# Luh1124/face-vae

Hardware: AMD Instinct MI355X
Metric: training images/sec (256x256 face-VAE step) (higher is better)
Workload: dtype bf16; 1 GPU; FaceVAE step 256x256 (AFE trunk + reparam + Generator trunk, MSE+KL, Adam); global_batch=32, per_gpu_batch=32, resolution=256, parallelism=dp1

## Files before the change

### face-vae_amd/_lib.py

```python
from __future__ import annotations

import ctypes
import os
from ctypes import POINTER, c_float, c_int, c_long, c_size_t, c_void_p

import torch

_HERE = os.path.dirname(os.path.realpath(__file__))
LIB_PATH = os.environ.get("FV_LIB_PATH") or os.path.join(_HERE, "libfacevae.so")

FV_F32, FV_BF16, FV_F64 = 0, 1, 2
FV_E_BADARG, FV_E_UNSUPPORTED, FV_E_COMM = 1001, 1002, 1003
ADAM_CHUNK = 4096
ABI_VERSION = 2


class ConvDesc(ctypes.Structure):
    _fields_ = [
        ("dtype", c_int), ("n", c_int), ("h", c_int), ("w", c_int),
        ("cin", c_int), ("cin_valid", c_int), ("cout", c_int), ("ldy", c_int),
        ("ksize", c_int), ("upsample", c_int), ("pro_act", c_int), ("pro_slope", c_float),
        ("epi_sigmoid", c_int), ("out_nchw_f32", c_int),
    ]

# ... 40 lines not shown
    "fv_conv_wt_elems": (c_size_t, [D]),
    "fv_conv2d_stats_blocks": (c_int, [D]),
    "fv_conv2d_stats_block_pixels": (c_int, [D]),
    "fv_conv_weight_prep": (c_int, [D, P, P, P, P, P]),
    "fv_conv2d_fwd": (c_int, [D, P, P, P, P, P, P, P, P, P]),
    "fv_conv2d_bwd_data": (c_int, [D, P, c_int, P, P, P]),
    "fv_conv2d_dgrad_lowres": (c_int, [D]),
    "fv_conv2d_wgrad_nsplit": (c_int, [D]),
    "fv_conv2d_wgrad_slab_elems": (c_size_t, [D]),
    "fv_conv2d_wgrad_bias_slab_elems": (c_size_t, [D]),
    "fv_conv2d_bwd_weight": (c_int, [D, P, P, P, P, c_int, P, P, P]),
    "fv_conv2d_wgrad_reduce": (c_int, [D, P, P, P, P, P]),
    "fv_conv2d_sr_records": (c_int, [D, c_int, POINTER(c_int)]),
    "fv_conv2d_fwd_sr": (c_int, [D, P, P, P, P, P, P, P]),
    "fv_conv2d_bwd_data_sr": (c_int, [D, P, c_int, P, P, P, P]),
    "fv_bn_bwd_from_records": (c_int, [P, c_int, c_int, c_long, c_int, c_long, P, P, P, P, P, P]),
    "fv_convt_supported": (c_int, [D]),
    "fv_convt_weight_prep": (c_int, [D, P, c_int, c_float, P, P, P, P]),
    "fv_convt_wgrad_reduce": (c_int, [D, P, P, P, c_int, c_float, P, P, P, P]),
    "fv_convt_eff_weight": (c_int, [P, c_int, c_int, c_int, c_int, c_float, P, P, P]),
    "fv_convt_weight_grad": (c_int, [P, c_int, c_int, c_int, c_int, c_float, P, P, P]),
    "fv_convt_direct_fwd": (c_int, [c_int, P, c_int, c_int, c_int, c_int, c_int, P, P, c_int, c_int, c_int, c_int,
                                    c_int, P, P]),
    "fv_convt_direct_dgrad": (c_int, [c_int, P, c_int, c_int, c_int, c_int, c_int, P, c_int, c_int, c_int, c_int,
                                      c_int, P, P]),
    "fv_convt_direct_wgrad": (c_int, [c_int, P, P, c_int, c_int, c_int, c_int, c_int, c_int, c_int, c_int, c_int,
                                      c_int, P, P, P]),
    "fv_chan_scale_fwd": (c_int, [c_int, P, c_int, c_long, c_int, c_int, P, P, P, P]),
    "fv_chan_scale_bwd": (c_int, [c_int, P, P, c_int, c_long, c_int, c_int, P, P, P, P, P]),
    "fv_fp8_ws_bytes": (c_size_t, []),
# ... 315 lines not shown
```

### face-vae_amd/csrc/conv.hip

```cpp
#include "conv_plan.h"

namespace {

__global__ void weight_prep_c7n_kernel(const float* __restrict__ wp, const float* sigma, bf16* wn, int cout) {
  const float inv = sigma ? 1.f / sigma[0] : 1.f;
  for (int e = blockIdx.x * blockDim.x + threadIdx.x; e < 32 * 448; e += gridDim.x * blockDim.x) {
    const int nn = e / 448, k = e - nn * 448;
    const int co = nn / 7, s = nn - co * 7, r = k >> 6, ci = k & 63;
    const float v = co < cout ? wp[((co * 64 + ci) * 7 + r) * 7 + s] * inv : 0.f;
    wn[e] = (bf16)v;
  }
}

template <typename T>
__device__ __forceinline__ void weight_prep_body(const float* __restrict__ wp, const float* sigma, T* wk, int rows,
                                                 int Kpad, int cout, int cin_valid, int lgCin, int KS, int K,
                                                 int transposed, int bid, int nblk, int smaj = 0) {
  const int total = rows * Kpad;
  const float inv = sigma ? 1.f / sigma[0] : 1.f;
  for (int e = bid * (int)blockDim.x + threadIdx.x; e < total; e += nblk * (int)blockDim.x) {
    int row, k;
    bool kin;
    int tap, c;
    if (smaj == 2) {
// ... 843 lines not shown
  }
  const bool c64 = use_c64(d);
  if (c64 && !res && !a.spm) {
    if ((st = wext(d->cout, kpad_of(3, 64), "c64"))) return st;
    const int nb = c64_bands(d);
    const int nblk = d->n * (d->w / 64) * (d->cout / 64) * nb;
    const unsigned xb = (unsigned)((long)d->n * d->h * d->w * 64 * 2);
    launch_c64(a, nblk, xb, nb, s);
    return fv_check_launch("conv2d_fwd_c64");
  }
  if (use_c74(d)) {
    FV_REQUIRE(!res, "packed 7x7 conv: no residual");
    const int ntiles = d->n * (d->h / C74_TR) * (d->w / 64);
    const unsigned xb = (unsigned)((long)d->n * d->h * d->w * d->cin * 2);
    FV_REQUIRE(!a.stats || a.nrec == c74_grid(d), "packed 7x7 conv: %d BN records for %d blocks", a.nrec, c74_grid(d));
    launch_c74(a, c74_grid(d), xb, ntiles, s);
    return fv_check_launch("conv2d_fwd_c74");
  }
  if (const int tr = halo_tr(d)) {
    if ((st = wext(plan_tile(d).bn, kpad_of(7, d->cin), "halo7"))) return st;
    a.lgtw = 6;
    const int nblk = d->n * (d->h / tr) * (d->w / 64);
    const unsigned xb = (unsigned)((long)d->n * d->h * d->w * d->cin * 2);
    if (launch_halo7(a, d->cin, nblk, xb, s)) {
      fv_set_error("7x7 halo conv variant unsupported (cin=%d)", d->cin);
      return FV_E_BADARG;
    }
    return fv_check_launch("conv2d_fwd_halo");
  }
  if (use_upband(d)) {
    FV_REQUIRE(!res && !a.spm, "sub-pixel band conv: no residual / store-pass records");
// ... 124 lines not shown
  return conv_run(d, x, wk, bias, pro_scale, pro_shift, res, y, stats, (hipStream_t)stream);
}

static fv_conv_desc dgrad_desc(const fv_conv_desc* d) {
  fv_conv_desc t{};
  t.dtype = d->dtype;
  t.n = d->n; t.h = d->h; t.w = d->w;
  t.cin = pad_pow2_8(d->cout);
  t.cin_valid = d->cout;
  t.cout = d->cin;
  t.ldy = d->cin;
  t.ksize = d->ksize;
  return t;
}

int fv_conv2d_sr_records(const fv_conv_desc* d, int dgrad, int* record_pixels) {
  if (check_desc(d) != FV_OK) return 0;
  if (dgrad) {
    if (d->upsample) return 0;
    const fv_conv_desc t = dgrad_desc(d);
    return sr_geometry(&t, record_pixels);
  }
  return sr_geometry(d, record_pixels);
}

int fv_conv2d_fwd_sr(const fv_conv_desc* d, const void* x, const void* wk, const float* bias, const void* res, void* y,
                     const fv_store_reduce* sr, void* stream) {
  int st = check_desc(d);
  if (st) return st;
  FV_REQUIRE(x && wk && y && sr && sr->mode == 1, "fwd_sr: null pointer or mode != 1");
  FV_REQUIRE(!d->pro_act && !d->out_nchw_f32 && d->ldy == d->cout, "fwd_sr: plain NHWC output only");
  return conv_run(d, x, wk, bias, nullptr, nullptr, res, y, nullptr, (hipStream_t)stream, sr);
}

int fv_conv2d_bwd_data_sr(const fv_conv_desc* d, const void* dy, int ldy_dy, const void* wt, void* dx,
                          const fv_store_reduce* sr, void* stream) {
  int st = check_desc(d);
  if (st) return st;
  FV_REQUIRE(dy && wt && dx && sr && sr->mode == 2 && !d->upsample, "bwd_data_sr: bad argument");
  const fv_conv_desc t = dgrad_desc(d);
  FV_REQUIRE(ldy_dy == t.cin, "bwd_data: dy channel stride must be %d (got %d)", t.cin, ldy_dy);
  return conv_run(&t, dy, wt, nullptr, nullptr, nullptr, nullptr, dx, nullptr, (hipStream_t)stream, sr);
}

int fv_conv2d_bwd_data(const fv_conv_desc* d, const void* dy, int ldy_dy, const void* wt, void* dx,
                       void* stream) {
  int st = check_desc(d);
  if (st) return st;
  const fv_conv_desc t = dgrad_desc(d);
  FV_REQUIRE(ldy_dy == t.cin, "bwd_data: dy channel stride must be %d (got %d)", t.cin, ldy_dy);
  if (const int bn = dgrad_halo_bn(d)) {
    FV_REQUIRE(dy && wt && dx, "null pointer");
    ConvArgs a{};
    a.x = dy; a.w = wt; a.y = dx;
    a.N = d->n; a.H = d->h / 2; a.W = d->w / 2; a.Hin = d->h; a.Win = d->w;
    a.Ho = a.H; a.Wo = a.W;
    a.P = d->n * a.H * a.W;
// ... 1447 lines not shown
```

### face-vae_amd/csrc/conv_plan.h

```cpp
#pragma once
#include "conv_common.h"

#pragma GCC visibility push(hidden)

constexpr int C74_TR = 4;
constexpr int C74_K = 224;
constexpr int C64_G = 8;
constexpr int UPB_G = 4;
constexpr int C7_TR = 4;

int launch_halo3_fwd3(const ConvArgs& a, int bn, int mode, int sch, bool pers, int grid, unsigned xb, int ntiles,
                      hipStream_t s);
int launch_halo3_fwd2(const ConvArgs& a, int bn, int nblk, unsigned xb, hipStream_t s);

int launch_halo7(const ConvArgs& a, int cin, int nblk, unsigned xb, hipStream_t s);
void launch_c74(const ConvArgs& a, int grid, unsigned xb, int ntiles, hipStream_t s);
void launch_c64(const ConvArgs& a, int nblk, unsigned xb, int nbands, hipStream_t s);
void launch_upband(const ConvArgs& a, int nblk, unsigned xb, int nbands, hipStream_t s);
int launch_c1s(const ConvArgs& a, int k, int bpx, int grid, unsigned xb, hipStream_t s);
void launch_c7n(const ConvArgs& a, int nblk, unsigned xb, int band, hipStream_t s);

struct WgArgs {
  const void* x;
  const float* psc;
  const float* psh;
  float slope;
  const void* dy;
  float* slab;
  float* bslab;
  int N, H, W, Hin, Win, P;
  int lgCin, Cin;
// ... 98 lines not shown
```

### face-vae_amd/csrc/conv_shapes.hip

```cpp
#include "conv_plan.h"

namespace {

template <int KS, int CIN, int RN, int TR, bool WLDS, bool KSPLIT>
__global__ void __launch_bounds__(512, 4)
conv_halo_fwd(ConvArgs a, unsigned x_bytes) {
  constexpr int PAD = KS / 2, TW = 64;
  constexpr int MT = TR * 4;
  constexpr int RM = KSPLIT ? MT : MT / 8;
  constexpr int HR = TR + KS - 1, HW = TW + KS - 1;
  constexpr int CPP = CIN / 8;
  constexpr int HCH = HR * HW * CPP;
  constexpr int HQ = (HCH + 63) / 64;
  constexpr int KPAD = ((KS * KS * CIN + 31) / 32) * 32;
  constexpr int NKS = KPAD / 32;
  constexpr int KPW = (NKS + 7) / 8;
  constexpr int WROW = KPAD / 8 + 1;
  constexpr int WCH = RN * 16 * WROW;
  constexpr int WQ = WLDS ? (WCH + 63) / 64 : 0;
  constexpr int HB = HQ * 1024, WB = WQ * 1024;
  constexpr int SCR = 4096;
  static_assert(!KSPLIT || (RN == 1 && !WLDS && 8 * MT * 1024 <= HB), "k-split layout");
  __shared__ __attribute__((aligned(1024))) char smem[HB + WB + SCR];
  char* halo = smem;
// ... 103 lines not shown
    __syncthreads();
    f32x4 t[1][1];
    t[0][0] = f32x4{0.f, 0.f, 0.f, 0.f};
#pragma unroll
    for (int w = 0; w < 8; ++w) t[0][0] += red[(w * RM + wave) * 64 + lane];
    conv_epilogue<bf16, 1, 8, 1, 1>(a, t, smem + HB + WB, 0, p0, tile, 0, wave, lane, tid);
  } else {
    conv_epilogue<bf16, 1, 8, RN, RM>(a, acc, smem + HB + WB, 0, p0, tile, 0, wave, lane, tid);
  }
}

constexpr int C74_HW = 71, C74_HR = C74_TR + 6;
constexpr int C74_WCOL = C74_K / 8;
constexpr int C74_WQ = 64 * C74_WCOL / 64;
constexpr int C74_HQ = (C74_HR * C74_HW + 63) / 64;
__global__ void __launch_bounds__(512, 2)
conv7c4_fwd(ConvArgs a, unsigned x_bytes, int ntiles) {
  constexpr int WB = C74_WQ * 1024, HB = C74_HQ * 1024, NHB = 3;
  __shared__ __attribute__((aligned(1024))) char smem[WB + NHB * HB];
  const int tid = threadIdx.x, lane = tid & 63;
  const int wave = __builtin_amdgcn_readfirstlane(tid >> 6);
  const int li = lane & 15, g = lane >> 4;
  const int tiles_w = a.W >> 6, tiles_h = a.H / C74_TR;
  const unsigned sbase = __builtin_amdgcn_readfirstlane((unsigned)(size_t)(lds_ptr_t)smem);
  const __amdgpu_buffer_rsrc_t xr = __builtin_amdgcn_make_buffer_rsrc(const_cast<void*>(a.x), 0, (int)x_bytes, 0x00020000);
  const __amdgpu_buffer_rsrc_t wr = __builtin_amdgcn_make_buffer_rsrc(const_cast<void*>(a.w), 0, 0x7fffffff, 0x00020000);

  auto issue_halo = [&](int tile, int buf) {
    const int n = tile / (tiles_h * tiles_w), rem = tile - n * tiles_h * tiles_w;
    const int h0 = (rem / tiles_w) * C74_TR, w0 = (rem % tiles_w) * 64;
    for (int q = wave; q < C74_HQ; q += 8) {
      const int L = q * 64 + lane;
      const int hr = L / C74_HW, hc = L - (L / C74_HW) * C74_HW;
      const int hh = h0 + hr - 3, ww = w0 + hc - 3;
      const bool ok = L < C74_HR * C74_HW && hh >= 0 && hh < a.H && ww >= 0 && ww < a.W;
      dma16s(xr, sbase + WB + buf * HB + q * 1024, ok ? (unsigned)((((n * a.H + hh) * a.W + ww) * 8) * 2) : 0x80000000u, 0u);
    }
  };
  for (int q = wave; q < C74_WQ; q += 8) {
    const int L = q * 64 + lane;
    const int li = L & 15, t = L >> 4, col = t % C74_WCOL, row = (t / C74_WCOL) * 16 + li;
    dma16s(wr, sbase + q * 1024, (unsigned)((row * C74_K + col * 8) * 2), 0u);
  }
  int tile = blockIdx.x;
  if (tile < ntiles) issue_halo(tile, 0);
  if (tile + (int)gridDim.x < ntiles) issue_halo(tile + gridDim.x, 1);
  asm volatile("s_waitcnt vmcnt(0)" ::: "memory");
  __syncthreads();

  float bv[4][4];
#pragma unroll
  for (int nn = 0; nn < 4; ++nn)
#pragma unroll
    for (int i = 0; i < 4; ++i) bv[nn][i] = a.bias ? a.bias[nn * 16 + g * 4 + i] : 0.f;
  int hbase[2];
#pragma unroll
  for (int m = 0; m < 2; ++m) {
    const int loc = wave * 32 + m * 16 + li;
    hbase[m] = (loc >> 6) * C74_HW + (loc & 63);
  }
  float bs[4][4], bq[4][4];
#pragma unroll
  for (int nn = 0; nn < 4; ++nn)
#pragma unroll
    for (int i = 0; i < 4; ++i) bs[nn][i] = bq[nn][i] = 0.f;
  int buf = 0;
  for (; tile < ntiles; tile += gridDim.x) {
    const int ahead = tile + 2 * gridDim.x;
    if (ahead < ntiles) issue_halo(ahead, buf == 0 ? 2 : buf - 1);
    f32x4 acc[4][2];
#pragma unroll
    for (int nn = 0; nn < 4; ++nn)
#pragma unroll
      for (int m = 0; m < 2; ++m) acc[nn][m] = f32x4{0.f, 0.f, 0.f, 0.f};
    const char* hs = smem + WB + buf * HB;
#pragma unroll
    for (int r = 0; r < 7; ++r) {
      bf16x8 bfr[4], afr[2];
#pragma unroll
      for (int nn = 0; nn < 4; ++nn)
        bfr[nn] = *reinterpret_cast<const bf16x8*>(smem + ((nn * C74_WCOL + r * 4 + g) * 16 + li) * 16);
#pragma unroll
      for (int m = 0; m < 2; ++m) {
        const char* p = hs + (hbase[m] + r * C74_HW + 2 * g) * 16;
        const uint2 lo = *reinterpret_cast<const uint2*>(p), hi = *reinterpret_cast<const uint2*>(p + 16);
        afr[m] = __builtin_bit_cast(bf16x8, make_uint4(lo.x, lo.y, hi.x, hi.y));
      }
#pragma unroll
      for (int nn = 0; nn < 4; ++nn)
#pragma unroll
        for (int m = 0; m < 2; ++m) acc[nn][m] = __builtin_amdgcn_mfma_f32_16x16x32_bf16(bfr[nn], afr[m], acc[nn][m], 0, 0, 0);
    }
    const int n = tile / (tiles_h * tiles_w), rem = tile - n * tiles_h * tiles_w;
    const int p0 = (n * a.H + (rem / tiles_w) * C74_TR) * a.W + (rem % tiles_w) * 64;
#pragma unroll
    for (int nn = 0; nn < 4; ++nn)
#pragma unroll
      for (int m = 0; m < 2; ++m)
#pragma unroll
        for (int i = 0; i < 4; ++i) acc[nn][m][i] += bv[nn][i];
    if (a.stats) {
#pragma unroll
      for (int nn = 0; nn < 4; ++nn)
#pragma unroll
        for (int i = 0; i < 4; ++i) {
          const float v0 = acc[nn][0][i], v1 = acc[nn][1][i];
          bs[nn][i] += v0 + v1;
          bq[nn][i] += v0 * v0 + v1 * v1;
        }
    }
    auto pk = [](float lo, float hi) {
      const bf16 t[2] = {(bf16)lo, (bf16)hi};
      return *reinterpret_cast<const unsigned*>(t);
    };
#pragma unroll
    for (int m = 0; m < 2; ++m) {
      const int loc = wave * 32 + m * 16 + li;
      bf16* yp = reinterpret_cast<bf16*>(a.y) + (long)(p0 + (loc >> 6) * a.W + (loc & 63)) * a.ldy;
#pragma unroll
      for (int q = 0; q < 2; ++q) {
        const f32x4 va = acc[2 * q][m], vb = acc[2 * q + 1][m];
        const auto s0 = __builtin_amdgcn_permlane16_swap(pk(va[0], va[1]), pk(vb[0], vb[1]), false, false);
        const auto s1 = __builtin_amdgcn_permlane16_swap(pk(va[2], va[3]), pk(vb[2], vb[3]), false, false);
        *reinterpret_cast<uint4*>(yp + (2 * q + (g & 1)) * 16 + (g >> 1) * 8) = make_uint4(s0[0], s1[0], s0[1], s1[1]);
      }
    }
    {
      const int dpieces = ahead < ntiles ? (wave + 8 < C74_HQ ? 2 : 1) : 0;
      wait_vm_dyn(8 + dpieces);
    }
    wait_lgkm0();
    __builtin_amdgcn_s_barrier();
    asm volatile("" ::: "memory");
    buf = buf == 2 ? 0 : buf + 1;
  }
  if (a.stats) {
    float* sw = reinterpret_cast<float*>(smem + WB);
#pragma unroll
    for (int nn = 0; nn < 4; ++nn)
#pragma unroll
      for (int i = 0; i < 4; ++i) {
        const float sv = row16_sum(bs[nn][i]), qv = row16_sum(bq[nn][i]);
        if (li == 0) {
          sw[wave * 128 + nn * 16 + g * 4 + i] = sv;
          sw[wave * 128 + 64 + nn * 16 + g * 4 + i] = qv;
        }
      }
    __syncthreads();
    if (tid < 128 && (int)blockIdx.x < a.nrec) {
      float v = 0.f;
#pragma unroll
      for (int w = 0; w < 8; ++w) v += sw[w * 128 + tid];
      a.stats[(long)blockIdx.x * 128 + tid] = v;
    }
  }
}

constexpr int C64_PXB = 160, C64_ROWB = 11 * 1024, C64_NR = 10;
__global__ void __launch_bounds__(512, 1)
conv3c64_fwd(ConvArgs a, unsigned x_bytes, int nbands) {
  __shared__ __attribute__((aligned(1024))) char smem[C64_NR * C64_ROWB];
  __shared__ __attribute__((aligned(16))) float sbias[64];
  __shared__ __attribute__((aligned(16))) float sacc[8 * 16 * 64];
  const int tid = threadIdx.x, lane = tid & 63;
  const int wave = __builtin_amdgcn_readfirstlane(tid >> 6);
  const int cg = wave & 1, rw = wave >> 1;
  const int lr = lane & 15, lh = lane >> 4;
  const int nblk = gridDim.x, bid = blockIdx.x;
// ... 520 lines not shown
      else reinterpret_cast<bf16*>(a.y)[((long)n * HWo + pix) * a.ldy + co] = (bf16)v;
    }
  }
}


}

int launch_halo7(const ConvArgs& a, int cin, int nblk, unsigned xb, hipStream_t s) {
  if (cin == 8) hipLaunchKernelGGL((conv_halo_fwd<7, 8, 4, 4, true, false>), dim3(nblk), dim3(512), 0, s, a, xb);
  else if (cin == 64) hipLaunchKernelGGL((conv_halo_fwd<7, 64, 1, 2, false, true>), dim3(nblk), dim3(512), 0, s, a, xb);
  else return FV_E_UNSUPPORTED;
  return FV_OK;
}

void launch_c74(const ConvArgs& a, int grid, unsigned xb, int ntiles, hipStream_t s) {
  hipLaunchKernelGGL(conv7c4_fwd, dim3(grid), dim3(512), 0, s, a, xb, ntiles);
}

void launch_c64(const ConvArgs& a, int nblk, unsigned xb, int nbands, hipStream_t s) {
  hipLaunchKernelGGL(conv3c64_fwd, dim3(nblk), dim3(512), 0, s, a, xb, nbands);
}

void launch_upband(const ConvArgs& a, int nblk, unsigned xb, int nbands, hipStream_t s) {
  hipLaunchKernelGGL(conv3up_band_fwd, dim3(nblk), dim3(512), 0, s, a, xb, nbands);
}

int launch_c1s(const ConvArgs& a, int k, int bpx, int grid, unsigned xb, hipStream_t s) {
  if (k == 256 && bpx == 128) hipLaunchKernelGGL((conv1x1_stream<256, 128>), dim3(grid), dim3(512), 0, s, a, xb);
  else if (k == 256 && bpx == 64) hipLaunchKernelGGL((conv1x1_stream<256, 64>), dim3(grid), dim3(512), 0, s, a, xb);
  else if (k == 512 && bpx == 64) hipLaunchKernelGGL((conv1x1_stream<512, 64>), dim3(grid), dim3(512), 0, s, a, xb);
  else if (k == 512 && bpx == 32) hipLaunchKernelGGL((conv1x1_stream<512, 32>), dim3(grid), dim3(512), 0, s, a, xb);
// ... 8 lines not shown
```

### face-vae_amd/ops.py

```python
from __future__ import annotations

import ctypes
import os
import weakref
from typing import Optional

import torch

from . import _lib as L
from ._lib import call, ptr, query, stream

CL = torch.channels_last
F32 = torch.float32
F64 = torch.float64
FP8 = torch.float8_e4m3fn
_FP8_HANDOFF = True


def storage(mode: torch.dtype) -> torch.dtype:
    return torch.bfloat16 if mode == FP8 else mode


def fp8_site(conv, which: str, device):
    sites = conv.__dict__.setdefault("_fv_fp8_sites", {})
# ... 345 lines not shown
        return part
    _timed("fwd", d, lambda: call("fv_conv2d_fwd", ctypes.byref(d), ptr(x), ptr(cs.wk), ptr(bias), ptr(psc),
                                  ptr(psh), ptr(res), ptr(y), ptr(part), stream()))
    if CHECK is not None:
        CHECK("fwd", cs, x=x, bias=bias, pro=pro, res=res, y=y)
    return part


def sr_records(d, dgrad):
    bp = ctypes.c_int(0)
    nrec = query("fv_conv2d_sr_records", ctypes.byref(d), int(dgrad), ctypes.byref(bp))
    return (nrec, bp.value) if nrec > 0 else None


class BNRecords:
    __slots__ = ("part", "nb", "bp", "dx")

    def __init__(self, part, nb, bp, dx):
        self.part, self.nb, self.bp, self.dx = part, nb, bp, dx


def _dgrad_bnred(cs, dy, dx, bnred):
    d = cs.d
    if bnred is None or cs.fp8 or d.upsample or d.dtype != L.FV_BF16:
        return None
    geo = sr_records(d, True)
    if geo is None:
        return None
    bn, r, ybn, slope = bnred
    if r.count == 0 and r.stats is None:
        return None
    nb, bp = geo
    part = _empty(nb * 2 * d.cin, F32, dy.device)
    sr = L.StoreReduce(2, ptr(part), ptr(ybn), ptr(r.mean), ptr(r.invstd), ptr(bn.weight), ptr(bn.bias),
                       float(slope))
    _timed("dgrad", d, lambda: call("fv_conv2d_bwd_data_sr", ctypes.byref(d), ptr(dy), d.cout, ptr(cs.wt), ptr(dx),
                                    ctypes.byref(sr), stream()))
    return BNRecords(part, nb, bp, dx)

# ... 260 lines not shown
def bn_backward_is_local(r: BNResult, comm) -> bool:
    return comm is None or (r.count == 0 and r.stats is None)


def bn_act_backward(dout, y, bn, r: BNResult, slope, pool, comm, addend=None, need_dx=True, recs=None, q8=None,
                    only8=False):
    N, C, H, W = y.shape
    dev = y.device
    dc = L.dtype_code(y.dtype)
    if bn_backward_is_local(r, comm):
        comm = None
    ws = _empty(query("fv_bn_ws_bytes", C) // 8, F64, dev)
    dg = torch.empty(C, dtype=F32, device=dev)
    dbt = torch.empty(C, dtype=F32, device=dev)
    k = torch.empty(2 * C, dtype=F32, device=dev)
    if recs is not None and not pool and recs.dx.data_ptr() == dout.data_ptr():
        P = N * H * W
        if comm is None:
            call("fv_bn_bwd_from_records", ptr(recs.part), recs.nb, recs.bp, P, C, int(r.count), ptr(dg), ptr(dbt),
                 ptr(k), None, ptr(ws), stream())
        else:
            red = torch.empty(2 * C, dtype=F64, device=dev)
            call("fv_bn_bwd_from_records", ptr(recs.part), recs.nb, recs.bp, P, C, 0, ptr(dg), ptr(dbt), None,
                 ptr(red), ptr(ws), stream())
            if need_dx:
                _sync(red, comm)
                call("fv_bn_bwd_finalize_dev", ptr(red), C, ptr(r.stats), None, None, ptr(k), stream())
    elif comm is None:
        evalm = r.count == 0 and r.stats is None
        call("fv_bn_act_bwd_reduce_finalize", dc, ptr(dout), ptr(y), N, H, W, C, C, ptr(r.mean), ptr(r.invstd),
# ... 10 lines not shown
            _sync(red, comm)
            call("fv_bn_bwd_finalize_dev", ptr(red), C, ptr(r.stats), None, None, ptr(k), stream())
    dx = q = None
    if need_dx:
        q8ok = _q8_ok(q8, y, pool, bn)
        if q8ok and only8:
            dx = torch.empty(0, dtype=y.dtype, device=dev)
        else:
            dx = torch.empty((N, C, H, W), dtype=y.dtype, device=dev, memory_format=CL)
        if q8ok:
            dx8 = _empty(N * C * H * W, torch.uint8, dev)
            call("fv_bn_act_bwd_apply_q8", dc, ptr(dout), ptr(y), N, H, W, C, ptr(r.mean), ptr(r.invstd),
                 ptr(bn.weight), ptr(bn.bias), float(slope), ptr(k), ptr(addend), None if only8 else ptr(dx),
                 ptr(dx8), ptr(q8[0]), stream())
            q = (dx8, q8[0][18:19].view(F32))
        else:
            call("fv_bn_act_bwd_apply", dc, ptr(dout), ptr(y), N, H, W, C, C, ptr(r.mean), ptr(r.invstd),
                 ptr(bn.weight), ptr(bn.bias), float(slope), int(pool), ptr(k), ptr(addend), ptr(dx), stream())
    if CHECK is not None and comm is None:
        CHECK("bn_bwd", bn, dout=dout, y=y, r=r, slope=slope, pool=pool, addend=addend, dx=dx, dg=dg, dbt=dbt)
    return (dx, dg, dbt, q) if q8 is not None else (dx, dg, dbt)


def grad_in(g: torch.Tensor, dtype) -> torch.Tensor:
    return g.to(dtype).contiguous(memory_format=CL)



class ConvBNActFn(torch.autograd.Function):

    @staticmethod
    def forward(ctx, x, weight, bias, gamma, beta, blk):
        mode = blk.compute_dtype()
# ... 13 lines not shown
        comm = blk.bn_comm()
        r = bn_from_partials(bn, part, cs, True, comm) if training else bn_finalize(bn, None, 0, False)
        z = bn_act_forward(y, r, blk.slope, blk.pool, bn)
        cs.release()
        ctx.blk, ctx.cs, ctx.r, ctx.comm = blk, cs, r, comm
        ctx.holder = {"bn": bn, "r": r, "y": y, "slope": blk.slope, "pool": blk.pool, "nuse": 0}
        blk._fv_holder = ctx.holder if training else None
        ctx.src = _claim_bnsrc(x, xb)
        ctx.save_for_backward(x, xb, y)
        return z

    @staticmethod
    def backward(ctx, dz):
        x, xb, y = ctx.saved_tensors
        blk, cs, r = ctx.blk, ctx.cs, ctx.r
        dz = grad_in(dz, y.dtype)
        recs = ctx.holder.get("recs") if ctx.holder["nuse"] == 1 else None
        q8 = fp8_site(cs.conv, "dy", y.device) if cs.fp8 and not blk.pool else None
        out = bn_act_backward(dz, y, blk.bn, r, blk.slope, blk.pool, ctx.comm, recs=recs, q8=q8)
        dy, dg, dbt = out[:3]
        dxb, dw, db, recs_in = conv_backward(cs, xb, dy, y.shape[1], need_dx=ctx.needs_input_grad[0],
                                             bnred=_bnred_of(ctx.src), want_recs=True,
                                             dy8=out[3] if q8 is not None else None)
        if ctx.src is not None:
            ctx.src["recs"] = recs_in
        dx = from_nhwc(dxb, x) if dxb is not None else None
        return dx, dw, db, dg, dbt, None


def _claim_bnsrc(x, xb):
    src = getattr(x, "_fv_bnsrc", None)
    if src is None or src[1] != x._version:
        return None
# ... 136 lines not shown
    def forward(ctx, x, weight, bias, conv, mode, sigmoid):
        dtype = storage(mode)
        xb, cin_pad = to_nhwc(x, dtype)
        N, _, H, W = x.shape
        cout = conv.out_channels
        nchw = bool(sigmoid) or (cout % 8 != 0)
        d = desc(dtype, N, H, W, cin_pad, conv.in_channels, cout, cout, conv.kernel_size, sig=sigmoid, nchw=nchw)
        cs = ConvState(conv, d, dtype, x.device, conv.training, need_wt=ctx.needs_input_grad[0], fp8=mode == FP8)
        if nchw:
            y = torch.empty((N, cout, H, W), dtype=F32, device=x.device)
        else:
            y = torch.empty((N, cout, H, W), dtype=dtype, device=x.device, memory_format=CL)
        conv_forward(cs, xb, bias, y=y)
        cs.release()
        ctx.cs, ctx.sigmoid, ctx.nchw, ctx.dtype = cs, sigmoid, nchw, dtype
        ctx.save_for_backward(x, xb, y if sigmoid else None)
        return y

    @staticmethod
    def backward(ctx, dy):
        x, xb, y = ctx.saved_tensors
        cs = ctx.cs
        d = cs.d
        dtype = ctx.dtype
        if ctx.nchw:
            ldd = pad_pow2(d.cout)
            dpre = torch.empty((d.n, ldd, d.h, d.w), dtype=dtype, device=dy.device, memory_format=CL)
            dy32 = dy.float().contiguous()
            if ctx.sigmoid:
                call("fv_sigmoid_bwd_to_nhwc", L.dtype_code(dtype), ptr(dy32), ptr(y), d.n, d.cout, d.h * d.w, ldd,
                     ptr(dpre), stream())
            else:
                call("fv_nchw_to_nhwc", L.dtype_code(dtype), ptr(dy32), d.n, d.cout, d.h * d.w, ldd, ptr(dpre),
                     stream())
        else:
            ldd = d.cout
            dpre = grad_in(dy, dtype)
        dxb, dw, db = conv_backward(cs, xb, dpre, ldd, need_dx=ctx.needs_input_grad[0])
        dx = from_nhwc(dxb, x) if dxb is not None else None
        return dx, dw, db, None, None, None



class S2ConvState:

    def __init__(self, conv, d, in_hw, dtype, device, training, need_wt):
        self.conv, self.d, self.in_hw = conv, d, in_hw
        w = conv.weight_param()
        if w.dtype != F32 or not w.is_contiguous():
            raise RuntimeError("conv weights must be contiguous fp32")
        self.w = w
        self.sigma = None
        self.fp8 = False
# ... 389 lines not shown
```

### include/facevae.h

```cpp
#ifndef FACEVAE_H
#define FACEVAE_H

#include <stddef.h>
#include <stdint.h>

#ifdef __cplusplus
extern "C" {
#endif

#define FV_ABI_VERSION 2

enum fv_status {
  FV_OK = 0,
  FV_E_BADARG = 1001,
  FV_E_UNSUPPORTED = 1002,
  FV_E_COMM = 1003
};

enum fv_dtype { FV_F32 = 0, FV_BF16 = 1, FV_F64 = 2 };

int fv_abi_version(void);
const char* fv_last_error(void);

typedef struct fv_conv_desc {
// ... 55 lines not shown
int fv_conv2d_s2_wgrad_reduce(const fv_conv_desc* d, const float* slab, const float* bias_slab, float* dw_param,
                              float* db, void* stream);

typedef struct fv_store_reduce {
  int mode;
  float* records;
  const void* bn_input;
  const float *mean, *invstd, *gamma, *beta;
  float slope;
} fv_store_reduce;
int fv_conv2d_sr_records(const fv_conv_desc* d, int dgrad, int* record_pixels);
int fv_conv2d_fwd_sr(const fv_conv_desc* d, const void* x, const void* wk, const float* bias, const void* res, void* y,
                     const fv_store_reduce* sr, void* stream);
int fv_conv2d_bwd_data_sr(const fv_conv_desc* d, const void* dy, int ldy_dy, const void* wt, void* dx,
                          const fv_store_reduce* sr, void* stream);
int fv_bn_bwd_from_records(const float* records, int nrec, int record_pixels, long pixels, int c, long count,
                           float* dgamma, float* dbeta, float* k, double* red, void* ws, void* stream);

int fv_convt_supported(const fv_conv_desc* d);
int fv_convt_weight_prep(const fv_conv_desc* d, const float* w, int demod, float gain, float* inv,
                         void* wk, void* wt, void* stream);
int fv_convt_wgrad_reduce(const fv_conv_desc* d, const float* slab, const float* bias_slab,
                          const float* w, int demod, float gain, const float* inv, float* dw,
                          float* db, void* stream);

int fv_convt_eff_weight(const float* w, int cin, int cout, int k, int demod, float gain, float* inv, float* we,
                        void* stream);
int fv_convt_weight_grad(const float* w, int cin, int cout, int k, int demod, float gain, const float* inv, float* g,
                         void* stream);
int fv_convt_direct_fwd(int dtype, const void* x, int n, int hi, int wi, int cin, int ldx, const float* we,
// ... 352 lines not shown
```

Baseline: 2859 images/s.

## Fuse output 7x7 conv data-gradient with BN-activation backward, recomputing instead of storing dx

For the final 7x7 output conv, the data gradient is no longer written to memory. One kernel pass (EPI=1) computes the dgrad and reduces the BN backward sums into per-block records. A second pass (EPI=2) recomputes the dgrad and applies the BN/leaky-ReLU backward directly to produce the input gradient. This removes the write and read of the full-resolution dx tensor and the separate BN apply kernel, at the cost of running the 7x7 MFMA convolution twice. Python autograd passes a placeholder gradient tensor and falls back to an explicit dgrad when the placeholder is not consumed directly.

New measurement: 2882 images/s (median of 6 runs). About the same (+0.8%).

```diff
diff --git a/face-vae_amd/_lib.py b/face-vae_amd/_lib.py
--- a/face-vae_amd/_lib.py
+++ b/face-vae_amd/_lib.py
@@ -78,6 +78,7 @@
     "fv_conv2d_sr_records": (c_int, [D, c_int, POINTER(c_int)]),
     "fv_conv2d_fwd_sr": (c_int, [D, P, P, P, P, P, P, P]),
     "fv_conv2d_bwd_data_sr": (c_int, [D, P, c_int, P, P, P, P]),
+    "fv_conv2d_bwd_data_bnapply": (c_int, [D, P, c_int, P, P, P, P, P]),
     "fv_bn_bwd_from_records": (c_int, [P, c_int, c_int, c_long, c_int, c_long, P, P, P, P, P, P]),
     "fv_convt_supported": (c_int, [D]),
     "fv_convt_weight_prep": (c_int, [D, P, c_int, c_float, P, P, P, P]),
diff --git a/face-vae_amd/csrc/conv.hip b/face-vae_amd/csrc/conv.hip
--- a/face-vae_amd/csrc/conv.hip
+++ b/face-vae_amd/csrc/conv.hip
@@ -881,7 +881,7 @@
     const int ntiles = d->n * (d->h / C74_TR) * (d->w / 64);
     const unsigned xb = (unsigned)((long)d->n * d->h * d->w * d->cin * 2);
     FV_REQUIRE(!a.stats || a.nrec == c74_grid(d), "packed 7x7 conv: %d BN records for %d blocks", a.nrec, c74_grid(d));
-    launch_c74(a, c74_grid(d), xb, ntiles, s);
+    launch_c74(a, 0, c74_grid(d), xb, ntiles, s);
     return fv_check_launch("conv2d_fwd_c74");
   }
   if (const int tr = halo_tr(d)) {
@@ -1036,11 +1036,41 @@
   return t;
 }
 
+static bool c74_bnbwd_ok(const fv_conv_desc* t) {
+  if (!use_c74(t)) return false;
+  if ((long)t->n * t->h * t->w * t->ldy * 2 >= (1L << 31)) return false;
+  return (t->n * (t->h / C74_TR) * (t->w / 64)) % c74_tiles_per_block(t) == 0;
+}
+
+static int c74_bnbwd_run(const fv_conv_desc* t, int epi, const void* dy, const void* wt, const fv_store_reduce* sr,
+                         const float* k, void* dx_bn, hipStream_t s) {
+  FV_REQUIRE(sr->bn_input && sr->mean && sr->invstd && sr->gamma && sr->beta, "packed 7x7 BN backward: null BN argument");
+  FV_REQUIRE(epi == 1 ? sr->records != nullptr : (k && dx_bn), "packed 7x7 BN backward: null output / k");
+  ConvArgs a{};
+  a.x = dy; a.w = wt; a.res = sr->bn_input; a.y = dx_bn;
+  a.sprec = epi == 1 ? sr->records : nullptr;
+  a.bnm = sr->mean; a.bni = sr->invstd; a.bng = sr->gamma; a.bnb = sr->beta; a.bns = sr->slope;
+  a.psc = k; a.psh = k ? k + 64 : nullptr;
+  a.N = t->n; a.H = t->h; a.W = t->w; a.Hin = t->h; a.Win = t->w;
+  a.P = t->n * t->h * t->w;
+  a.Cin = t->cin; a.lgCin = fv_ilog2(t->cin);
+  a.Cout = t->cout; a.ldy = t->ldy;
+  a.nrec = c74_grid(t);
+  const int ntiles = t->n * (t->h / C74_TR) * (t->w / 64);
+  const unsigned xb = (unsigned)((long)t->n * t->h * t->w * t->cin * 2);
+  launch_c74(a, epi, c74_grid(t), xb, ntiles, s);
+  return fv_check_launch(epi == 1 ? "conv2d_bwd_data_c74_bnsums" : "conv2d_bwd_data_c74_bnapply");
+}
+
 int fv_conv2d_sr_records(const fv_conv_desc* d, int dgrad, int* record_pixels) {
   if (check_desc(d) != FV_OK) return 0;
   if (dgrad) {
     if (d->upsample) return 0;
     const fv_conv_desc t = dgrad_desc(d);
+    if (c74_bnbwd_ok(&t)) {
+      if (record_pixels) *record_pixels = c74_tiles_per_block(&t) * C74_TR * 64;
+      return c74_grid(&t);
+    }
     return sr_geometry(&t, record_pixels);
   }
   return sr_geometry(d, record_pixels);
@@ -1059,10 +1089,35 @@
                           const fv_store_reduce* sr, void* stream) {
   int st = check_desc(d);
   if (st) return st;
-  FV_REQUIRE(dy && wt && dx && sr && sr->mode == 2 && !d->upsample, "bwd_data_sr: bad argument");
+  FV_REQUIRE(dy && wt && sr && sr->mode == 2 && !d->upsample, "bwd_data_sr: bad argument");
   const fv_conv_desc t = dgrad_desc(d);
   FV_REQUIRE(ldy_dy == t.cin, "bwd_data: dy channel stride must be %d (got %d)", t.cin, ldy_dy);
+  if (c74_bnbwd_ok(&t)) {
+    if (dx) {
+      fv_set_error("bwd_data_sr: the packed 7x7 data gradient writes records only (dx must be NULL)");
+      return FV_E_UNSUPPORTED;
+    }
+    return c74_bnbwd_run(&t, 1, dy, wt, sr, nullptr, nullptr, (hipStream_t)stream);
+  }
+  if (!dx) {
+    fv_set_error("bwd_data_sr: dx == NULL (records only) is the packed 7x7 data gradient's form");
+    return FV_E_UNSUPPORTED;
+  }
   return conv_run(&t, dy, wt, nullptr, nullptr, nullptr, nullptr, dx, nullptr, (hipStream_t)stream, sr);
+}
+
+int fv_conv2d_bwd_data_bnapply(const fv_conv_desc* d, const void* dy, int ldy_dy, const void* wt,
+                               const fv_store_reduce* sr, const float* k, void* dx_bn, void* stream) {
+  int st = check_desc(d);
+  if (st) return st;
+  FV_REQUIRE(dy && wt && sr && sr->mode == 2 && k && dx_bn && !d->upsample, "bwd_data_bnapply: bad argument");
+  const fv_conv_desc t = dgrad_desc(d);
+  FV_REQUIRE(ldy_dy == t.cin, "bwd_data: dy channel stride must be %d (got %d)", t.cin, ldy_dy);
+  if (!c74_bnbwd_ok(&t)) {
+    fv_set_error("bwd_data_bnapply: only the packed 7x7 data gradient (fv_conv2d_sr_records) has this form");
+    return FV_E_UNSUPPORTED;
+  }
+  return c74_bnbwd_run(&t, 2, dy, wt, sr, k, dx_bn, (hipStream_t)stream);
 }
 
 int fv_conv2d_bwd_data(const fv_conv_desc* d, const void* dy, int ldy_dy, const void* wt, void* dx,
diff --git a/face-vae_amd/csrc/conv_plan.h b/face-vae_amd/csrc/conv_plan.h
--- a/face-vae_amd/csrc/conv_plan.h
+++ b/face-vae_amd/csrc/conv_plan.h
@@ -14,7 +14,7 @@
 int launch_halo3_fwd2(const ConvArgs& a, int bn, int nblk, unsigned xb, hipStream_t s);
 
 int launch_halo7(const ConvArgs& a, int cin, int nblk, unsigned xb, hipStream_t s);
-void launch_c74(const ConvArgs& a, int grid, unsigned xb, int ntiles, hipStream_t s);
+void launch_c74(const ConvArgs& a, int epi, int grid, unsigned xb, int ntiles, hipStream_t s);
 void launch_c64(const ConvArgs& a, int nblk, unsigned xb, int nbands, hipStream_t s);
 void launch_upband(const ConvArgs& a, int nblk, unsigned xb, int nbands, hipStream_t s);
 int launch_c1s(const ConvArgs& a, int k, int bpx, int grid, unsigned xb, hipStream_t s);
diff --git a/face-vae_amd/csrc/conv_shapes.hip b/face-vae_amd/csrc/conv_shapes.hip
--- a/face-vae_amd/csrc/conv_shapes.hip
+++ b/face-vae_amd/csrc/conv_shapes.hip
@@ -141,10 +141,18 @@
 constexpr int C74_WCOL = C74_K / 8;
 constexpr int C74_WQ = 64 * C74_WCOL / 64;
 constexpr int C74_HQ = (C74_HR * C74_HW + 63) / 64;
-__global__ void __launch_bounds__(512, 2)
+__device__ __forceinline__ float par8_sum(float v) {
+  v += dpp_f<0x4E>(v);
+  v += dpp_f<0x124>(v);
+  v += dpp_f<0x128>(v);
+  return v;
+}
+template <int EPI>
+__global__ void __launch_bounds__(512, EPI == 1 ? 4 : 2)
 conv7c4_fwd(ConvArgs a, unsigned x_bytes, int ntiles) {
   constexpr int WB = C74_WQ * 1024, HB = C74_HQ * 1024, NHB = 3;
-  __shared__ __attribute__((aligned(1024))) char smem[WB + NHB * HB];
+  constexpr int CB = EPI ? 6 * 64 * 4 : 0;
+  __shared__ __attribute__((aligned(1024))) char smem[WB + NHB * HB + CB];
   const int tid = threadIdx.x, lane = tid & 63;
   const int wave = __builtin_amdgcn_readfirstlane(tid >> 6);
   const int li = lane & 15, g = lane >> 4;
@@ -172,6 +180,39 @@
   int tile = blockIdx.x;
   if (tile < ntiles) issue_halo(tile, 0);
   if (tile + (int)gridDim.x < ntiles) issue_halo(tile + gridDim.x, 1);
+  uint4 uv[2][2];
+  auto chunk_off = [&](int t, int m, int q) {
+    t = min(t, ntiles - 1);
+    const int n = t / (tiles_h * tiles_w), rem = t - n * tiles_h * tiles_w;
+    const int p0 = (n * a.H + (rem / tiles_w) * C74_TR) * a.W + (rem % tiles_w) * 64;
+    const int loc = wave * 32 + m * 16 + li;
+    return (unsigned)(p0 + (loc >> 6) * a.W + (loc & 63)) * 128u + (unsigned)((2 * q + (g & 1)) * 32 + (g >> 1) * 16);
+  };
+  auto load_u = [&](int t, int q) {
+#pragma unroll
+    for (int m = 0; m < 2; ++m)
+      uv[m][q] = *reinterpret_cast<const uint4*>(reinterpret_cast<const char*>(a.res) + chunk_off(t, m, q));
+  };
+  if constexpr (EPI != 0) {
+    if (ntiles > 0) {
+      load_u(tile, 0);
+      load_u(tile, 1);
+    }
+  }
+  const float* const cst = reinterpret_cast<const float*>(smem + WB + NHB * HB);
+  if constexpr (EPI != 0) {
+    float* cw = reinterpret_cast<float*>(smem + WB + NHB * HB);
+    if (tid < 64) {
+      cw[tid] = a.bnm[tid];
+      cw[64 + tid] = a.bni[tid];
+      cw[128 + tid] = a.bng[tid];
+      cw[192 + tid] = a.bnb[tid];
+      if constexpr (EPI == 2) {
+        cw[256 + tid] = a.psc[tid];
+        cw[320 + tid] = a.psh[tid];
+      }
+    }
+  }
   asm volatile("s_waitcnt vmcnt(0)" ::: "memory");
   __syncthreads();
 
@@ -179,7 +220,7 @@
 #pragma unroll
   for (int nn = 0; nn < 4; ++nn)
 #pragma unroll
-    for (int i = 0; i < 4; ++i) bv[nn][i] = a.bias ? a.bias[nn * 16 + g * 4 + i] : 0.f;
+    for (int i = 0; i < 4; ++i) bv[nn][i] = (EPI == 0 && a.bias) ? a.bias[nn * 16 + g * 4 + i] : 0.f;
   int hbase[2];
 #pragma unroll
   for (int m = 0; m < 2; ++m) {
@@ -201,32 +242,59 @@
 #pragma unroll
       for (int m = 0; m < 2; ++m) acc[nn][m] = f32x4{0.f, 0.f, 0.f, 0.f};
     const char* hs = smem + WB + buf * HB;
-#pragma unroll
-    for (int r = 0; r < 7; ++r) {
-      bf16x8 bfr[4], afr[2];
-#pragma unroll
-      for (int nn = 0; nn < 4; ++nn)
-        bfr[nn] = *reinterpret_cast<const bf16x8*>(smem + ((nn * C74_WCOL + r * 4 + g) * 16 + li) * 16);
-#pragma unroll
-      for (int m = 0; m < 2; ++m) {
-        const char* p = hs + (hbase[m] + r * C74_HW + 2 * g) * 16;
-        const uint2 lo = *reinterpret_cast<const uint2*>(p), hi = *reinterpret_cast<const uint2*>(p + 16);
-        afr[m] = __builtin_bit_cast(bf16x8, make_uint4(lo.x, lo.y, hi.x, hi.y));
-      }
-#pragma unroll
-      for (int nn = 0; nn < 4; ++nn)
-#pragma unroll
-        for (int m = 0; m < 2; ++m) acc[nn][m] = __builtin_amdgcn_mfma_f32_16x16x32_bf16(bfr[nn], afr[m], acc[nn][m], 0, 0, 0);
-    }
+    if constexpr (EPI != 1) {
+#pragma unroll
+      for (int r = 0; r < 7; ++r) {
+        bf16x8 bfr[4], afr[2];
+#pragma unroll
+        for (int nn = 0; nn < 4; ++nn)
+          bfr[nn] = *reinterpret_cast<const bf16x8*>(smem + ((nn * C74_WCOL + r * 4 + g) * 16 + li) * 16);
+#pragma unroll
+        for (int m = 0; m < 2; ++m) {
+          const char* p = hs + (hbase[m] + r * C74_HW + 2 * g) * 16;
+          const uint2 lo = *reinterpret_cast<const uint2*>(p), hi = *reinterpret_cast<const uint2*>(p + 16);
+          afr[m] = __builtin_bit_cast(bf16x8, make_uint4(lo.x, lo.y, hi.x, hi.y));
+        }
+#pragma unroll
+        for (int nn = 0; nn < 4; ++nn)
+#pragma unroll
+          for (int m = 0; m < 2; ++m) acc[nn][m] = __builtin_amdgcn_mfma_f32_16x16x32_bf16(bfr[nn], afr[m], acc[nn][m], 0, 0, 0);
+      }
+      if constexpr (EPI == 2) __builtin_amdgcn_sched_barrier(0);
+    }
+    auto mma2 = [&](auto nt0c) {
+      constexpr int nt0 = decltype(nt0c)::value;
+#pragma unroll
+      for (int r = 0; r < 7; ++r) {
+        bf16x8 bfr[2], afr[2];
+#pragma unroll
+        for (int nn = 0; nn < 2; ++nn)
+          bfr[nn] = *reinterpret_cast<const bf16x8*>(smem + (((nt0 + nn) * C74_WCOL + r * 4 + g) * 16 + li) * 16);
+#pragma unroll
+        for (int m = 0; m < 2; ++m) {
+          const char* p = hs + (hbase[m] + r * C74_HW + 2 * g) * 16;
+          const uint2 lo = *reinterpret_cast<const uint2*>(p), hi = *reinterpret_cast<const uint2*>(p + 16);
+          afr[m] = __builtin_bit_cast(bf16x8, make_uint4(lo.x, lo.y, hi.x, hi.y));
+        }
+#pragma unroll
+        for (int nn = 0; nn < 2; ++nn)
+#pragma unroll
+          for (int m = 0; m < 2; ++m)
+            acc[nt0 + nn][m] = __builtin_amdgcn_mfma_f32_16x16x32_bf16(bfr[nn], afr[m], acc[nt0 + nn][m], 0, 0, 0);
+        __builtin_amdgcn_sched_barrier(0);
+      }
+    };
     const int n = tile / (tiles_h * tiles_w), rem = tile - n * tiles_h * tiles_w;
     const int p0 = (n * a.H + (rem / tiles_w) * C74_TR) * a.W + (rem % tiles_w) * 64;
-#pragma unroll
-    for (int nn = 0; nn < 4; ++nn)
-#pragma unroll
-      for (int m = 0; m < 2; ++m)
-#pragma unroll
-        for (int i = 0; i < 4; ++i) acc[nn][m][i] += bv[nn][i];
-    if (a.stats) {
+    if constexpr (EPI == 0) {
+#pragma unroll
+      for (int nn = 0; nn < 4; ++nn)
+#pragma unroll
+        for (int m = 0; m < 2; ++m)
+#pragma unroll
+          for (int i = 0; i < 4; ++i) acc[nn][m][i] += bv[nn][i];
+    }
+    if (EPI == 0 && a.stats) {
 #pragma unroll
       for (int nn = 0; nn < 4; ++nn)
 #pragma unroll
@@ -240,37 +308,119 @@
       const bf16 t[2] = {(bf16)lo, (bf16)hi};
       return *reinterpret_cast<const unsigned*>(t);
     };
-#pragma unroll
-    for (int m = 0; m < 2; ++m) {
-      const int loc = wave * 32 + m * 16 + li;
-      bf16* yp = reinterpret_cast<bf16*>(a.y) + (long)(p0 + (loc >> 6) * a.W + (loc & 63)) * a.ldy;
-#pragma unroll
-      for (int q = 0; q < 2; ++q) {
-        const f32x4 va = acc[2 * q][m], vb = acc[2 * q + 1][m];
-        const auto s0 = __builtin_amdgcn_permlane16_swap(pk(va[0], va[1]), pk(vb[0], vb[1]), false, false);
-        const auto s1 = __builtin_amdgcn_permlane16_swap(pk(va[2], va[3]), pk(vb[2], vb[3]), false, false);
-        *reinterpret_cast<uint4*>(yp + (2 * q + (g & 1)) * 16 + (g >> 1) * 8) = make_uint4(s0[0], s1[0], s0[1], s1[1]);
+    if constexpr (EPI == 0) {
+#pragma unroll
+      for (int m = 0; m < 2; ++m) {
+        const int loc = wave * 32 + m * 16 + li;
+        bf16* yp = reinterpret_cast<bf16*>(a.y) + (long)(p0 + (loc >> 6) * a.W + (loc & 63)) * a.ldy;
+#pragma unroll
+        for (int q = 0; q < 2; ++q) {
+          const f32x4 va = acc[2 * q][m], vb = acc[2 * q + 1][m];
+          const auto s0 = __builtin_amdgcn_permlane16_swap(pk(va[0], va[1]), pk(vb[0], vb[1]), false, false);
+          const auto s1 = __builtin_amdgcn_permlane16_swap(pk(va[2], va[3]), pk(vb[2], vb[3]), false, false);
+          *reinterpret_cast<uint4*>(yp + (2 * q + (g & 1)) * 16 + (g >> 1) * 8) = make_uint4(s0[0], s1[0], s0[1], s1[1]);
+        }
+      }
+    } else {
+      auto epi_q = [&](auto qc) {
+        constexpr int q = decltype(qc)::value;
+        int c0 = (2 * q + (g & 1)) * 16 + (g >> 1) * 8;
+        asm volatile("" : "+v"(c0));
+        unsigned dw[2][4], ow[2][4];
+        float tg[2][4] = {}, ty[2][4] = {};
+#pragma unroll
+        for (int m = 0; m < 2; ++m) {
+          const f32x4 va = acc[2 * q][m], vb = acc[2 * q + 1][m];
+          const auto s0 = __builtin_amdgcn_permlane16_swap(pk(va[0], va[1]), pk(vb[0], vb[1]), false, false);
+          const auto s1 = __builtin_amdgcn_permlane16_swap(pk(va[2], va[3]), pk(vb[2], vb[3]), false, false);
+          dw[m][0] = s0[0]; dw[m][1] = s1[0]; dw[m][2] = s0[1]; dw[m][3] = s1[1];
+        }
+#pragma unroll
+        for (int h = 0; h < 2; ++h) {
+          const f32x4 mean = *reinterpret_cast<const f32x4*>(cst + c0 + 4 * h);
+          const f32x4 inv = *reinterpret_cast<const f32x4*>(cst + 64 + c0 + 4 * h);
+          const f32x4 gam = *reinterpret_cast<const f32x4*>(cst + 128 + c0 + 4 * h);
+          const f32x4 bet = *reinterpret_cast<const f32x4*>(cst + 192 + c0 + 4 * h);
+          f32x4 k0 = {0.f, 0.f, 0.f, 0.f}, k1 = {0.f, 0.f, 0.f, 0.f};
+          if constexpr (EPI == 2) {
+            k0 = *reinterpret_cast<const f32x4*>(cst + 256 + c0 + 4 * h);
+            k1 = *reinterpret_cast<const f32x4*>(cst + 320 + c0 + 4 * h);
+          }
+#pragma unroll
+          for (int m = 0; m < 2; ++m) {
+            const unsigned uw[4] = {uv[m][q].x, uv[m][q].y, uv[m][q].z, uv[m][q].w};
+            float o[4];
+#pragma unroll
+            for (int j = 0; j < 4; ++j) {
+              const unsigned dd = dw[m][2 * h + (j >> 1)], ud = uw[2 * h + (j >> 1)];
+              const float dv = __uint_as_float((j & 1) ? (dd & 0xffff0000u) : (dd << 16));
+              const float uf = __uint_as_float((j & 1) ? (ud & 0xffff0000u) : (ud << 16));
+              const float yh = (uf - mean[j]) * inv[j];
+              const float z = gam[j] * yh + bet[j];
+              const float gg = z > 0.f ? dv : dv * a.bns;
+              if constexpr (EPI == 1) {
+                tg[h][j] += gg;
+                ty[h][j] += gg * yh;
+              } else {
+                o[j] = gam[j] * inv[j] * (gg - k0[j] - yh * k1[j]);
+              }
+            }
+            if constexpr (EPI == 2) {
+              ow[m][2 * h] = pk(o[0], o[1]);
+              ow[m][2 * h + 1] = pk(o[2], o[3]);
+            }
+          }
+        }
+        if constexpr (EPI == 1) {
+#pragma unroll
+          for (int j = 0; j < 4; ++j) {
+            const bool odd = li & 1;
+            bs[q][j] += (odd ? tg[1][j] : tg[0][j]) + dpp_f<0xB1>(odd ? tg[0][j] : tg[1][j]);
+            bq[q][j] += (odd ? ty[1][j] : ty[0][j]) + dpp_f<0xB1>(odd ? ty[0][j] : ty[1][j]);
+          }
+        }
+        if constexpr (EPI == 2) {
+#pragma unroll
+          for (int m = 0; m < 2; ++m)
+            *reinterpret_cast<uint4*>(reinterpret_cast<char*>(a.y) + chunk_off(tile, m, q)) =
+                make_uint4(ow[m][0], ow[m][1], ow[m][2], ow[m][3]);
+        }
+        load_u(tile + gridDim.x, q);
+      };
+      if constexpr (EPI == 1) {
+        mma2(std::integral_constant<int, 0>{});
+        epi_q(std::integral_constant<int, 0>{});
+        __builtin_amdgcn_sched_barrier(0);
+        mma2(std::integral_constant<int, 2>{});
+        epi_q(std::integral_constant<int, 1>{});
+      } else {
+        epi_q(std::integral_constant<int, 0>{});
+        epi_q(std::integral_constant<int, 1>{});
       }
     }
     {
       const int dpieces = ahead < ntiles ? (wave + 8 < C74_HQ ? 2 : 1) : 0;
-      wait_vm_dyn(8 + dpieces);
+      wait_vm_dyn((EPI == 0 ? 8 : EPI == 1 ? 8 : 16) + dpieces);
     }
     wait_lgkm0();
     __builtin_amdgcn_s_barrier();
     asm volatile("" ::: "memory");
     buf = buf == 2 ? 0 : buf + 1;
   }
-  if (a.stats) {
+  float* const recs = EPI == 1 ? a.sprec : EPI == 0 ? a.stats : nullptr;
+  if (recs) {
     float* sw = reinterpret_cast<float*>(smem + WB);
 #pragma unroll
     for (int nn = 0; nn < 4; ++nn)
 #pragma unroll
       for (int i = 0; i < 4; ++i) {
-        const float sv = row16_sum(bs[nn][i]), qv = row16_sum(bq[nn][i]);
-        if (li == 0) {
-          sw[wave * 128 + nn * 16 + g * 4 + i] = sv;
-          sw[wave * 128 + 64 + nn * 16 + g * 4 + i] = qv;
+        if (EPI == 1 && nn >= 2) continue;
+        const float sv = EPI == 1 ? par8_sum(bs[nn][i]) : row16_sum(bs[nn][i]);
+        const float qv = EPI == 1 ? par8_sum(bq[nn][i]) : row16_sum(bq[nn][i]);
+        const int c = EPI == 1 ? (2 * nn + (g & 1)) * 16 + (g >> 1) * 8 + 4 * (li & 1) + i : nn * 16 + g * 4 + i;
+        if (EPI == 1 ? li < 2 : li == 0) {
+          sw[wave * 128 + c] = sv;
+          sw[wave * 128 + 64 + c] = qv;
         }
       }
     __syncthreads();
@@ -278,7 +428,7 @@
       float v = 0.f;
 #pragma unroll
       for (int w = 0; w < 8; ++w) v += sw[w * 128 + tid];
-      a.stats[(long)blockIdx.x * 128 + tid] = v;
+      recs[(long)blockIdx.x * 128 + tid] = v;
     }
   }
 }
@@ -829,8 +979,10 @@
   return FV_OK;
 }
 
-void launch_c74(const ConvArgs& a, int grid, unsigned xb, int ntiles, hipStream_t s) {
-  hipLaunchKernelGGL(conv7c4_fwd, dim3(grid), dim3(512), 0, s, a, xb, ntiles);
+void launch_c74(const ConvArgs& a, int epi, int grid, unsigned xb, int ntiles, hipStream_t s) {
+  if (epi == 1) hipLaunchKernelGGL(conv7c4_fwd<1>, dim3(grid), dim3(512), 0, s, a, xb, ntiles);
+  else if (epi == 2) hipLaunchKernelGGL(conv7c4_fwd<2>, dim3(grid), dim3(512), 0, s, a, xb, ntiles);
+  else hipLaunchKernelGGL(conv7c4_fwd<0>, dim3(grid), dim3(512), 0, s, a, xb, ntiles);
 }
 
 void launch_c64(const ConvArgs& a, int nblk, unsigned xb, int nbands, hipStream_t s) {
diff --git a/face-vae_amd/ops.py b/face-vae_amd/ops.py
--- a/face-vae_amd/ops.py
+++ b/face-vae_amd/ops.py
@@ -383,15 +383,42 @@
 
 
 class BNRecords:
-    __slots__ = ("part", "nb", "bp", "dx")
-
-    def __init__(self, part, nb, bp, dx):
-        self.part, self.nb, self.bp, self.dx = part, nb, bp, dx
+    __slots__ = ("part", "nb", "bp", "dx", "recipe")
+
+    def __init__(self, part, nb, bp, dx, recipe=None):
+        self.part, self.nb, self.bp, self.dx, self.recipe = part, nb, bp, dx, recipe
+
+    def is_placeholder(self, g):
+        return self.recipe is not None and g.data_ptr() == self.dx.data_ptr() and g.stride() == self.dx.stride() \
+            and g.dtype == self.dx.dtype
+
+
+OUTCONV_BNBWD = os.environ.get("FV_OUTCONV_BNBWD", "1") != "0"
+
+
+def _dgrad_bnsums(cs, dy, ldd, bnred):
+    d = cs.d
+    if not OUTCONV_BNBWD or bnred is None or cs.fp8 or d.upsample or d.dtype != L.FV_BF16 or d.ksize != 7:
+        return None
+    geo = sr_records(d, True)
+    if geo is None:
+        return None
+    bn, r, ybn, slope = bnred
+    if (r.count == 0 and r.stats is None) or ybn.dtype != dy.dtype or ybn.shape[1] != d.cin:
+        return None
+    nb, bp = geo
+    part = _empty(nb * 2 * d.cin, F32, dy.device)
+    sr = L.StoreReduce(2, ptr(part), ptr(ybn), ptr(r.mean), ptr(r.invstd), ptr(bn.weight), ptr(bn.bias),
+                       float(slope))
+    _timed("dgrad", d, lambda: call("fv_conv2d_bwd_data_sr", ctypes.byref(d), ptr(dy), ldd, ptr(cs.wt), None,
+                                    ctypes.byref(sr), stream()))
+    ph = torch.zeros(1, dtype=dy.dtype, device=dy.device).expand(d.n, d.cin, d.h, d.w)
+    return BNRecords(part, nb, bp, ph, (cs, dy, ldd))
 
 
 def _dgrad_bnred(cs, dy, dx, bnred):
     d = cs.d
-    if bnred is None or cs.fp8 or d.upsample or d.dtype != L.FV_BF16:
+    if bnred is None or cs.fp8 or d.upsample or d.dtype != L.FV_BF16 or d.ksize == 7:
         return None
     geo = sr_records(d, True)
     if geo is None:
@@ -682,6 +709,9 @@
     dg = torch.empty(C, dtype=F32, device=dev)
     dbt = torch.empty(C, dtype=F32, device=dev)
     k = torch.empty(2 * C, dtype=F32, device=dev)
+    fused = recs is not None and recs.recipe is not None
+    if fused and (pool or addend is not None or q8 is not None or not recs.is_placeholder(dout)):
+        raise RuntimeError("bn_act_backward: records of an unstored gradient need the plain apply form")
     if recs is not None and not pool and recs.dx.data_ptr() == dout.data_ptr():
         P = N * H * W
         if comm is None:
@@ -722,9 +752,17 @@
                  ptr(bn.weight), ptr(bn.bias), float(slope), ptr(k), ptr(addend), None if only8 else ptr(dx),
                  ptr(dx8), ptr(q8[0]), stream())
             q = (dx8, q8[0][18:19].view(F32))
+        elif fused:
+            cs2, dy2, ldd2 = recs.recipe
+            sr = L.StoreReduce(2, None, ptr(y), ptr(r.mean), ptr(r.invstd), ptr(bn.weight), ptr(bn.bias),
+                               float(slope))
+            call("fv_conv2d_bwd_data_bnapply", ctypes.byref(cs2.d), ptr(dy2), ldd2, ptr(cs2.wt), ctypes.byref(sr),
+                 ptr(k), ptr(dx), stream())
         else:
             call("fv_bn_act_bwd_apply", dc, ptr(dout), ptr(y), N, H, W, C, C, ptr(r.mean), ptr(r.invstd),
                  ptr(bn.weight), ptr(bn.bias), float(slope), int(pool), ptr(k), ptr(addend), ptr(dx), stream())
+    if CHECK is not None and fused:
+        dout, _ = _dgrad(*recs.recipe, True, None)
     if CHECK is not None and comm is None:
         CHECK("bn_bwd", bn, dout=dout, y=y, r=r, slope=slope, pool=pool, addend=addend, dx=dx, dg=dg, dbt=dbt)
     return (dx, dg, dbt, q) if q8 is not None else (dx, dg, dbt)
@@ -768,9 +806,18 @@
     def backward(ctx, dz):
         x, xb, y = ctx.saved_tensors
         blk, cs, r = ctx.blk, ctx.cs, ctx.r
-        dz = grad_in(dz, y.dtype)
         recs = ctx.holder.get("recs") if ctx.holder["nuse"] == 1 else None
         q8 = fp8_site(cs.conv, "dy", y.device) if cs.fp8 and not blk.pool else None
+        rec0 = ctx.holder.get("recs")
+        if rec0 is not None and rec0.recipe is not None:
+            if recs is not None and q8 is None and recs.is_placeholder(dz):
+                pass
+            else:
+                da, _ = _dgrad(*rec0.recipe[:3], True, None)
+                dz = grad_in(dz, y.dtype) + da
+                recs = None
+        else:
+            dz = grad_in(dz, y.dtype)
         out = bn_act_backward(dz, y, blk.bn, r, blk.slope, blk.pool, ctx.comm, recs=recs, q8=q8)
         dy, dg, dbt = out[:3]
         dxb, dw, db, recs_in = conv_backward(cs, xb, dy, y.shape[1], need_dx=ctx.needs_input_grad[0],
@@ -937,6 +984,7 @@
         conv_forward(cs, xb, bias, y=y)
         cs.release()
         ctx.cs, ctx.sigmoid, ctx.nchw, ctx.dtype = cs, sigmoid, nchw, dtype
+        ctx.src = _claim_bnsrc(x, xb)
         ctx.save_for_backward(x, xb, y if sigmoid else None)
         return y
 
@@ -959,7 +1007,17 @@
         else:
             ldd = d.cout
             dpre = grad_in(dy, dtype)
-        dxb, dw, db = conv_backward(cs, xb, dpre, ldd, need_dx=ctx.needs_input_grad[0])
+        src = ctx.src
+        recs = None
+        if ctx.needs_input_grad[0] and src is not None and not cs.fp8 and d.ksize == 7:
+            _, dw, db = conv_backward(cs, xb, dpre, ldd, need_dx=False)
+            recs = _dgrad_bnsums(cs, dpre, ldd, _bnred_of(src))
+            src["recs"] = recs
+            if recs is not None:
+                return recs.dx, dw, db, None, None, None
+            dxb, _ = _dgrad(cs, dpre, ldd, True, None)
+        else:
+            dxb, dw, db = conv_backward(cs, xb, dpre, ldd, need_dx=ctx.needs_input_grad[0])
         dx = from_nhwc(dxb, x) if dxb is not None else None
         return dx, dw, db, None, None, None
 
diff --git a/include/facevae.h b/include/facevae.h
--- a/include/facevae.h
+++ b/include/facevae.h
@@ -93,6 +93,8 @@
                      const fv_store_reduce* sr, void* stream);
 int fv_conv2d_bwd_data_sr(const fv_conv_desc* d, const void* dy, int ldy_dy, const void* wt, void* dx,
                           const fv_store_reduce* sr, void* stream);
+int fv_conv2d_bwd_data_bnapply(const fv_conv_desc* d, const void* dy, int ldy_dy, const void* wt,
+                               const fv_store_reduce* sr, const float* k, void* dx_bn, void* stream);
 int fv_bn_bwd_from_records(const float* records, int nrec, int record_pixels, long pixels, int c, long count,
                            float* dgamma, float* dbeta, float* k, double* red, void* ws, void* stream);
 
```
